# Vincentqyw/image-matching-webui

Hardware: AMD Instinct MI355X
Metric: image-pairs/sec @640x480 SuperPoint+LightGlue (higher is better)
Workload: dtype f32 via 3xf16 split MFMA, f32 accumulate; P.V of LightGlue's cross blocks in two products (audited per block: layer error <= 7.1e-6, score error <= 4.7e-5, profiles/r05_lab_attention_mix.txt)

## Files before the change

### image-matching-webui_amd/csrc/gemm_tile.h

```cpp
#pragma once
#include "gemm.h"

#define BM 128
#define BN 128

struct TileCtx {
    int M, N, row0, col0, seq, z;
    const float* bias;
    long wsel;
};

__device__ __forceinline__ bool gemm_tile_setup(const GemmP& p, TileCtx& c, int bn = BN, int bm = BM) {
    c.z = blockIdx.z;
    c.M = p.mcnt ? p.mcnt[c.z * p.cnt_stride] : p.M;
    c.N = p.ncnt ? p.ncnt[c.z * p.cnt_stride] : p.N;
    const int ncol = (p.N + bn - 1) / bn;
    const int tile = xcd_remap(blockIdx.x, gridDim.x);
    if (p.group_rows > 1) {
        const int nrow = (p.M + BM - 1) / BM;
        const int per = p.group_rows * ncol;
        const int g = tile / per, t = tile - g * per;
        const int rows = min(p.group_rows, nrow - g * p.group_rows);
        c.row0 = (g * p.group_rows + t % rows) * BM;
        c.col0 = (t / rows) * bn;
    } else {
        c.row0 = (tile / ncol) * bm;
        c.col0 = (tile % ncol) * bn;
    }
    if (c.row0 >= c.M || c.col0 >= c.N) return false;
    c.bias = p.bias;
    c.seq = 0;
    c.wsel = 0;
    if (p.rows_per_seq > 0) {
        c.seq = c.row0 / p.rows_per_seq;
        const int i0 = c.row0 - c.seq * p.rows_per_seq;
        if (p.cnt && i0 >= p.cnt[c.seq]) return false;
        if (p.active && p.active[c.seq >> 1] == 0) return false;
        if (p.wsel) {
            c.wsel = p.wsel[c.seq >> 1] + p.wsel_off;
            if (c.bias) c.bias += (size_t)c.wsel * p.b_stride;
        }
    }
    return true;
}
```

### image-matching-webui_amd/csrc/gemm_wreg.hip

```cpp
#include <stdlib.h>

#include "gemm.h"
#include "gemm_tile.h"

#define WR_BN 256
#ifdef WR_LAB
__device__ int wr_lab_flags = 0;
#define WR_FLAGS (__builtin_amdgcn_readfirstlane(wr_lab_flags))
#else
#define WR_FLAGS 0
#endif
#define WR_F_NOSTORE 1
#define WR_F_ONETILE 2
#define WR_F_NOEPI 4
#define WR_F_NOWLOAD 8
#define WR_F_NOXLOAD 16
#define WR_F_NOSTORE_V 32
#define WR_F_NOSTORE_QK 64
#define WR_F_STAGGER(f) (((f) >> 8) & 255)
#define WR_STG_ROW 68
#define WR_STG_TROW 36
#define WR_WAVE_LDS 9216

typedef unsigned int u32x4_t __attribute__((ext_vector_type(4)));
__device__ __forceinline__ const void* wr_uniform_ptr(const void* p) {
    const size_t v = (size_t)p;
    const unsigned lo32 = (unsigned)__builtin_amdgcn_readfirstlane((int)(unsigned)(v & 0xffffffffu));
    const unsigned hi32 = (unsigned)__builtin_amdgcn_readfirstlane((int)(unsigned)(v >> 32));
    return (const void*)((size_t)lo32 | ((size_t)hi32 << 32));
}
__device__ __forceinline__ void wr_wave_fence() {
    __builtin_amdgcn_s_waitcnt(0xc07f);
    __builtin_amdgcn_wave_barrier();
}

template <int EPI, bool SINGLE, bool PIPE = true, int MT = 4>
__global__ __launch_bounds__(256, 2) void gemm_wreg_kernel(GemmP p) {
    __shared__ uint4 smem[(4 * WR_WAVE_LDS) / 16];
    char* sm = reinterpret_cast<char*>(smem);
    const int tid = threadIdx.x;
    const int lane = tid & 63, wid = tid >> 6;
    const int lo = lane & 31, hi = lane >> 5;
    TileCtx c;
    if (!gemm_tile_setup(p, c, WR_BN, 32 * MT)) return;
    const float* A = p.A + (size_t)c.z * p.a_bs;
    const float wsc = p.wscale ? p.wscale[c.wsel] : 1.0f;
    const int labf = WR_FLAGS;
    if (WR_F_STAGGER(labf) != 0 && (int)blockIdx.x >= p.st_nct && (int)blockIdx.x < 4 * p.st_nct)
        for (int i = 0; i < WR_F_STAGGER(labf) * ((int)blockIdx.x / p.st_nct); ++i) __builtin_amdgcn_s_sleep(16);
    const int nkt = (labf & WR_F_ONETILE) ? 1 : p.K >> 5, nks = 2 * nkt;

    f32x16 acc[2][MT];
#pragma unroll
    for (int n = 0; n < 2; ++n)
#pragma unroll
        for (int m = 0; m < MT; ++m)
#pragma unroll
            for (int r = 0; r < 16; ++r) acc[n][m][r] = 0.0f;

    const int g = tid & 3;
    const int rl0 = tid >> 2, rl1 = 64 + (tid >> 2);
    const bool st0 = MT >= 2 || rl0 < 32, st1 = MT == 4;
    const int wo0 = (((g >> 1) * 4 + (rl0 >> 5)) * 64 + (g & 1) * 32 + ((rl0 & 31) ^ (2 * g))) * 16;
    const int wo1 = (((g >> 1) * 4 + (rl1 >> 5)) * 64 + (g & 1) * 32 + ((rl1 & 31) ^ (2 * g))) * 16;
    const float* pa0 = A + (size_t)min(c.row0 + (st0 ? rl0 : 0), c.M - 1) * p.lda + g * 8;
    const float* pa1 = A + (size_t)min(c.row0 + (st1 ? rl1 : 0), c.M - 1) * p.lda + g * 8;
    bool lnc = false;
    float mu0 = 0.f, mu1 = 0.f;
    if constexpr (EPI == EPI_QKV_VIT || EPI == EPI_CONV) {
        lnc = p.ln_stats != nullptr;
        if (lnc) {
            mu0 = p.ln_stats[2 * (size_t)min(c.row0 + (st0 ? rl0 : 0), c.M - 1)];
            mu1 = p.ln_stats[2 * (size_t)min(c.row0 + (st1 ? rl1 : 0), c.M - 1)];
        }
    }
    f32x4 xa0, xb0, xa1, xb1;
    auto issue = [&](int kt) __attribute__((always_inline)) {
        if (st0) {
            xa0 = *reinterpret_cast<const f32x4*>(pa0 + kt * 32);
            xb0 = *reinterpret_cast<const f32x4*>(pa0 + kt * 32 + 4);
        }
        if (st1) {
            xa1 = *reinterpret_cast<const f32x4*>(pa1 + kt * 32);
            xb1 = *reinterpret_cast<const f32x4*>(pa1 + kt * 32 + 4);
        }
    };
    auto store = [&](int stg) __attribute__((always_inline)) {
        uint4 h, l;
        if constexpr (EPI == EPI_QKV_VIT || EPI == EPI_CONV) {
            if (lnc) {
                xa0 -= mu0;
                xb0 -= mu0;
                xa1 -= mu1;
                xb1 -= mu1;
            }
        }
        if constexpr (SINGLE) {
            if (st0) *reinterpret_cast<uint4*>(sm + stg * 16384 + wo0) = half8_rtn(__builtin_bit_cast(float4, xa0), __builtin_bit_cast(float4, xb0));
            if (st1) *reinterpret_cast<uint4*>(sm + stg * 16384 + wo1) = half8_rtn(__builtin_bit_cast(float4, xa1), __builtin_bit_cast(float4, xb1));
            return;
        }
        if (st0) {
            split8(__builtin_bit_cast(float4, xa0), __builtin_bit_cast(float4, xb0), h, l);
            *reinterpret_cast<uint4*>(sm + stg * 16384 + wo0) = h;
            if constexpr (!SINGLE) *reinterpret_cast<uint4*>(sm + stg * 16384 + 8192 + wo0) = l;
        }
        if (st1) {
            split8(__builtin_bit_cast(float4, xa1), __builtin_bit_cast(float4, xb1), h, l);
            *reinterpret_cast<uint4*>(sm + stg * 16384 + wo1) = h;
            if constexpr (!SINGLE) *reinterpret_cast<uint4*>(sm + stg * 16384 + 8192 + wo1) = l;
        }
    };
    const int nfr = (p.N + 31) >> 5;
    const size_t plane_bytes = (size_t)nfr * 32 * p.K * 2;
    const __amdgpu_buffer_rsrc_t rWh =
        __builtin_amdgcn_make_buffer_rsrc(const_cast<void*>(wr_uniform_ptr(p.Wh + (size_t)c.wsel * p.w_stride)), 0, (unsigned)plane_bytes, 0x00020000);
    const __amdgpu_buffer_rsrc_t rWl =
        __builtin_amdgcn_make_buffer_rsrc(const_cast<void*>(wr_uniform_ptr(p.Wl + (size_t)c.wsel * p.w_stride)), 0, (unsigned)plane_bytes, 0x00020000);
    unsigned wof[2];
#pragma unroll
    for (int n = 0; n < 2; ++n) {
        const int nf = min((c.col0 >> 5) + 2 * wid + n, nfr - 1);
        wof[n] = (unsigned)((nf * (p.K >> 4)) * 64 + lane) * 16u;
    }
    uint4 wc[2][2], wn[2][2];
    auto loadw = [&](int s, uint4(&w)[2][2]) __attribute__((always_inline)) {
#pragma unroll
        for (int n = 0; n < 2; ++n) {
            const u32x4_t vh = __builtin_amdgcn_raw_buffer_load_b128(rWh, wof[n], (unsigned)s * 1024u, 0);
            w[n][0] = make_uint4(vh.x, vh.y, vh.z, vh.w);
            if constexpr (!SINGLE) {
                const u32x4_t vl = __builtin_amdgcn_raw_buffer_load_b128(rWl, wof[n], (unsigned)s * 1024u, 0);
                w[n][1] = make_uint4(vl.x, vl.y, vl.z, vl.w);
            }
        }
    };
    auto kstep = [&](int stg, int ks, uint4(&w)[2][2]) __attribute__((always_inline)) {
        const int apos = (hi * 32 + (lo ^ (2 * (2 * ks + hi)))) * 16;
#pragma unroll
        for (int mh = 0; mh < (MT + 1) / 2; ++mh) {
            constexpr int MH = MT >= 2 ? 2 : 1;
            uint4 ah[MH], al[MH];
#pragma unroll
            for (int m = 0; m < MH; ++m) {
                const int fo = stg * 16384 + (ks * 4 + 2 * mh + m) * 1024 + apos;
                ah[m] = *reinterpret_cast<const uint4*>(sm + fo);
                if constexpr (!SINGLE) al[m] = *reinterpret_cast<const uint4*>(sm + fo + 8192);
            }
#pragma unroll
            for (int n = 0; n < 2; ++n)
#pragma unroll
                for (int m = 0; m < MH; ++m) {
                    if constexpr (!SINGLE) {
                        acc[n][2 * mh + m] = mfma16(w[n][0], al[m], acc[n][2 * mh + m]);
                        acc[n][2 * mh + m] = mfma16(w[n][1], ah[m], acc[n][2 * mh + m]);
                    }
                    acc[n][2 * mh + m] = mfma16(w[n][0], ah[m], acc[n][2 * mh + m]);
                }
            if constexpr (PIPE) {
                if (mh == 0) __builtin_amdgcn_sched_barrier(0);
            }
        }
    };

    if constexpr (PIPE) {
        uint4 w0[2][2], w1[2][2], w2[2][2];
        issue(0);
        loadw(0, w0);
        if (nks > 1) loadw(1, w1);
        store(0);
        if (nkt > 1) issue(1);
        __syncthreads();
#define WR_TILE(KT, WA, WB, WC)                                  \
    {                                                            \
        const int kt_ = (KT), stg_ = kt_ & 1, s_ = 2 * kt_;      \
        if (s_ + 2 < nks && !(labf & WR_F_NOWLOAD)) loadw(s_ + 2, WC); \
        __builtin_amdgcn_sched_barrier(0);                       \
        kstep(stg_, 0, WA);                                      \
        __builtin_amdgcn_sched_barrier(0);                       \
        if (kt_ + 1 < nkt && !(labf & WR_F_NOXLOAD)) {           \
            store(stg_ ^ 1);                                     \
            if (kt_ + 2 < nkt) issue(kt_ + 2);                   \
        }                                                        \
        if (s_ + 3 < nks && !(labf & WR_F_NOWLOAD)) loadw(s_ + 3, WA); \
        __builtin_amdgcn_sched_barrier(0);                       \
        kstep(stg_, 1, WB);                                      \
        __syncthreads();                                         \
    }
        int kt = 0;
#pragma unroll 1
        for (; kt + 3 <= nkt; kt += 3) {
            WR_TILE(kt, w0, w1, w2)
            WR_TILE(kt + 1, w2, w0, w1)
            WR_TILE(kt + 2, w1, w2, w0)
        }
        if (kt < nkt) WR_TILE(kt, w0, w1, w2)
        if (kt + 1 < nkt) WR_TILE(kt + 1, w2, w0, w1)
#undef WR_TILE
    } else {
    issue(0);
    loadw(0, wc);
    store(0);
    if (nkt > 1) issue(1);
    __syncthreads();
#pragma unroll 1
    for (int kt = 0; kt < nkt; ++kt) {
        const int stg = kt & 1;
        loadw(2 * kt + 1, wn);
        kstep(stg, 0, wc);
        if (kt + 1 < nkt) {
            store(stg ^ 1);
            if (kt + 2 < nkt) issue(kt + 2);
            loadw(2 * kt + 2, wc);
        }
        kstep(stg, 1, wn);
        __syncthreads();
    }
    }

    float* st = reinterpret_cast<float*>(sm + wid * WR_WAVE_LDS);
    const int fw0 = c.col0 + 64 * wid;
    if (fw0 >= c.N) return;
    if (labf & WR_F_NOEPI) {
        if (acc[0][0][0] == 12345.678f) p.C[0] = acc[1][MT - 1][3];
        return;
    }
    bool do_store = !(labf & WR_F_NOSTORE);
    auto park_rows = [&](int m) __attribute__((always_inline)) {
#pragma unroll
        for (int n = 0; n < 2; ++n)
#pragma unroll
            for (int q = 0; q < 4; ++q)
                *reinterpret_cast<float4*>(st + lo * WR_STG_ROW + 32 * n + 8 * q + 4 * hi) =
                    make_float4(acc[n][m][4 * q + 0] * wsc, acc[n][m][4 * q + 1] * wsc, acc[n][m][4 * q + 2] * wsc, acc[n][m][4 * q + 3] * wsc);
    };
    if constexpr (EPI == EPI_QKV || EPI == EPI_CROSS || EPI == EPI_QKV_VIT) {
        const int CW = p.heads * 64;
        const int t = fw0 / CW, hd = (fw0 - t * CW) >> 6;
        float* dst;
        bool vt, rope, scale;
        if (EPI == EPI_QKV || EPI == EPI_QKV_VIT) {
            const int role = t + (EPI == EPI_QKV_VIT ? p.role0 : 0);
            dst = (role == 0) ? p.Q : (role == 1) ? p.Kt : p.V;
            vt = (role == 2);
            rope = (role < 2);
            scale = (role == 0);
        } else {
            dst = (t == 0) ? p.Q : p.V;
            vt = (t == 1);
            rope = false;
            scale = (t == 0);
        }
        unsigned short* d16 = reinterpret_cast<unsigned short*>(dst);
        if ((labf & WR_F_NOSTORE_V) && vt) do_store = false;
        if ((labf & WR_F_NOSTORE_QK) && !vt) do_store = false;
        const int R = p.rows_per_seq;
        const int i0 = c.row0 - c.seq * R;
        if (EPI == EPI_QKV_VIT && !vt) {
            const int tab0 = i0 + (p.rope_seq_row0 ? p.rope_seq_row0[c.seq] : 0);
            const int d0 = (lane & 7) * 8, dp = d0 ^ 16;
            const bool first = (d0 & 16) == 0;
            const int ti = (d0 >> 5) * 16 + (d0 & 8);
            float4 ba = make_float4(0.f, 0.f, 0.f, 0.f), bb = ba, pa = ba, pb = ba;
            if (c.bias != nullptr) {
                ba = *reinterpret_cast<const float4*>(c.bias + fw0 + d0);
                bb = *reinterpret_cast<const float4*>(c.bias + fw0 + d0 + 4);
                pa = *reinterpret_cast<const float4*>(c.bias + fw0 + dp);
                pb = *reinterpret_cast<const float4*>(c.bias + fw0 + dp + 4);
            }
#pragma unroll
            for (int m = 0; m < MT; ++m) {
                float4 tc[4][2], ts[4][2];
#pragma unroll
                for (int pass = 0; pass < 4; ++pass) {
                    const size_t ir = (size_t)(tab0 + 32 * m + pass * 8 + (lane >> 3)) * 32 + ti;
                    tc[pass][0] = *reinterpret_cast<const float4*>(p.rope_cos + ir);
                    tc[pass][1] = *reinterpret_cast<const float4*>(p.rope_cos + ir + 4);
                    ts[pass][0] = *reinterpret_cast<const float4*>(p.rope_sin + ir);
                    ts[pass][1] = *reinterpret_cast<const float4*>(p.rope_sin + ir + 4);
                }
                park_rows(m);
                wr_wave_fence();
#pragma unroll
                for (int pass = 0; pass < 4; ++pass) {
                    const int tl = pass * 8 + (lane >> 3);
                    const float4 va = *reinterpret_cast<const float4*>(st + tl * WR_STG_ROW + d0);
                    const float4 vb = *reinterpret_cast<const float4*>(st + tl * WR_STG_ROW + d0 + 4);
                    const float4 wa = *reinterpret_cast<const float4*>(st + tl * WR_STG_ROW + dp);
                    const float4 wb = *reinterpret_cast<const float4*>(st + tl * WR_STG_ROW + dp + 4);
                    float mine[8] = {va.x + ba.x, va.y + ba.y, va.z + ba.z, va.w + ba.w, vb.x + bb.x, vb.y + bb.y, vb.z + bb.z, vb.w + bb.w};
                    float part[8] = {wa.x + pa.x, wa.y + pa.y, wa.z + pa.z, wa.w + pa.w, wb.x + pb.x, wb.y + pb.y, wb.z + pb.z, wb.w + pb.w};
                    if (lnc) {
                        const float2 mr = *reinterpret_cast<const float2*>(p.ln_stats + 2 * (size_t)(c.row0 + 32 * m + tl));
                        const float xa[8] = {va.x, va.y, va.z, va.w, vb.x, vb.y, vb.z, vb.w}, xp[8] = {wa.x, wa.y, wa.z, wa.w, wb.x, wb.y, wb.z, wb.w};
                        const float ba8[8] = {ba.x, ba.y, ba.z, ba.w, bb.x, bb.y, bb.z, bb.w}, pa8[8] = {pa.x, pa.y, pa.z, pa.w, pb.x, pb.y, pb.z, pb.w};
#pragma unroll
                        for (int j = 0; j < 8; ++j) {
                            mine[j] = mr.y * xa[j] + ba8[j];
                            part[j] = mr.y * xp[j] + pa8[j];
                        }
                    }
                    const float cw[8] = {tc[pass][0].x, tc[pass][0].y, tc[pass][0].z, tc[pass][0].w, tc[pass][1].x, tc[pass][1].y, tc[pass][1].z, tc[pass][1].w};
                    const float ss[8] = {ts[pass][0].x, ts[pass][0].y, ts[pass][0].z, ts[pass][0].w, ts[pass][1].x, ts[pass][1].y, ts[pass][1].z, ts[pass][1].w};
                    float v[8];
#pragma unroll
                    for (int j = 0; j < 8; ++j) {
                        float x = mine[j], y = part[j];
                        asm volatile("" : "+v"(x), "+v"(y));
                        const float r = first ? __builtin_fmaf(x, cw[j], -(y * ss[j])) : __builtin_fmaf(x, cw[j], y * ss[j]);
                        v[j] = scale ? r * p.alpha : r;
                    }
                    uint4 hv, lv;
                    split8(make_float4(v[0], v[1], v[2], v[3]), make_float4(v[4], v[5], v[6], v[7]), hv, lv);
                    unsigned short* o = d16 + (((size_t)c.seq * p.heads + hd) * R + i0 + 32 * m + tl) * 64 + d0;
                    if (do_store) {
                        *reinterpret_cast<uint4*>(o) = hv;
                        *reinterpret_cast<uint4*>(o + p.plane_halves) = lv;
                    }
                }
                wr_wave_fence();
            }
        } else if (!vt) {
            const int d0 = (lane & 7) * 8;
            float4 ba = make_float4(0.f, 0.f, 0.f, 0.f), bb = ba;
            if (c.bias != nullptr) {
                ba = *reinterpret_cast<const float4*>(c.bias + fw0 + d0);
                bb = *reinterpret_cast<const float4*>(c.bias + fw0 + d0 + 4);
            }
            float4 tc[2][4], ts[2][4];
            auto load_tables = [&](int m, float4(&cs)[4], float4(&sn)[4]) __attribute__((always_inline)) {
#pragma unroll
                for (int pass = 0; pass < 4; ++pass) {
                    const size_t row = (size_t)(c.row0 + 32 * m + pass * 8 + (lane >> 3));
                    cs[pass] = *reinterpret_cast<const float4*>(p.rope_cos + row * 32 + (d0 >> 1));
                    sn[pass] = *reinterpret_cast<const float4*>(p.rope_sin + row * 32 + (d0 >> 1));
                }
            };
            if (rope) load_tables(0, tc[0], ts[0]);
#pragma unroll
            for (int m = 0; m < MT; ++m) {
                park_rows(m);
                wr_wave_fence();
                if (rope && m + 1 < MT) load_tables(m + 1, tc[(m + 1) & 1], ts[(m + 1) & 1]);
#pragma unroll
                for (int pass = 0; pass < 4; ++pass) {
                    const int tl = pass * 8 + (lane >> 3);
                    const float4 va = *reinterpret_cast<const float4*>(st + tl * WR_STG_ROW + d0);
                    const float4 vb = *reinterpret_cast<const float4*>(st + tl * WR_STG_ROW + d0 + 4);
                    float v[8] = {va.x + ba.x, va.y + ba.y, va.z + ba.z, va.w + ba.w, vb.x + bb.x, vb.y + bb.y, vb.z + bb.z, vb.w + bb.w};
                    if (rope) {
                        const float4 cs = tc[m & 1][pass], sn = ts[m & 1][pass];
                        const float cw[4] = {cs.x, cs.y, cs.z, cs.w}, ss[4] = {sn.x, sn.y, sn.z, sn.w};
#pragma unroll
                        for (int j = 0; j < 4; ++j) {
                            float a0 = v[2 * j], a1 = v[2 * j + 1];
                            asm volatile("" : "+v"(a0), "+v"(a1));
                            v[2 * j] = __builtin_fmaf(a0, cw[j], -(a1 * ss[j]));
                            v[2 * j + 1] = __builtin_fmaf(a1, cw[j], a0 * ss[j]);
                        }
                    }
                    if (scale) {
#pragma unroll
                        for (int j = 0; j < 8; ++j) v[j] *= p.alpha;
                    }
                    uint4 hv, lv;
                    split8(make_float4(v[0], v[1], v[2], v[3]), make_float4(v[4], v[5], v[6], v[7]), hv, lv);
                    unsigned short* o = d16 + (((size_t)c.seq * p.heads + hd) * R + i0 + 32 * m + tl) * 64 + d0;
                    if (do_store) {
                        *reinterpret_cast<uint4*>(o) = hv;
                        *reinterpret_cast<uint4*>(o + p.plane_halves) = lv;
                    }
                }
                wr_wave_fence();
            }
        } else {
#pragma unroll
            for (int m = 0; m < MT; ++m) {
#pragma unroll
                for (int n = 0; n < 2; ++n)
#pragma unroll
                    for (int r = 0; r < 16; ++r) st[(32 * n + 8 * (r >> 2) + 4 * hi + (r & 3)) * WR_STG_TROW + lo] = acc[n][m][r] * wsc;
                wr_wave_fence();
#pragma unroll
                for (int pass = 0; pass < 4; ++pass) {
                    const int d = pass * 16 + (lane >> 2), tk = (lane & 3) * 8;
                    const float bd = c.bias ? c.bias[fw0 + d] : 0.0f;
                    float4 va = *reinterpret_cast<const float4*>(st + d * WR_STG_TROW + tk);
                    float4 vb = *reinterpret_cast<const float4*>(st + d * WR_STG_TROW + tk + 4);
                    if (lnc) {
                        const float4* ms4 = reinterpret_cast<const float4*>(p.ln_stats + 2 * (size_t)(c.row0 + 32 * m + tk));
                        const float4 q0 = ms4[0], q1 = ms4[1], q2 = ms4[2], q3 = ms4[3];
                        va = make_float4(q0.y * va.x, q0.w * va.y, q1.y * va.z, q1.w * va.w);
                        vb = make_float4(q2.y * vb.x, q2.w * vb.y, q3.y * vb.z, q3.w * vb.w);
                    }
                    uint4 hv, lv;
                    split8(make_float4(va.x + bd, va.y + bd, va.z + bd, va.w + bd), make_float4(vb.x + bd, vb.y + bd, vb.z + bd, vb.w + bd), hv, lv);
                    unsigned short* o = d16 + (((size_t)c.seq * p.heads + hd) * 64 + d) * R + i0 + 32 * m + tk;
                    if (do_store) {
                        *reinterpret_cast<uint4*>(o) = hv;
                        *reinterpret_cast<uint4*>(o + p.plane_halves) = lv;
                    }
                }
                wr_wave_fence();
            }
        }
    } else {
        float* C = p.C + (size_t)c.z * p.c_bs;
        const int fl = (lane & 15) * 4;
        const int f0 = fw0 + fl;
        float4 b4 = make_float4(0.f, 0.f, 0.f, 0.f);
        if (c.bias != nullptr) b4 = *reinterpret_cast<const float4*>(c.bias + f0);
#pragma unroll
        for (int m = 0; m < MT; ++m) {
            park_rows(m);
            wr_wave_fence();
#pragma unroll
            for (int pass = 0; pass < 8; ++pass) {
                const int tl = pass * 4 + (lane >> 4);
                const int row = c.row0 + 32 * m + tl;
                if (row < c.M) {
                    float4 t4 = *reinterpret_cast<const float4*>(st + tl * WR_STG_ROW + fl);
                    if (lnc) {
                        const float rs = p.ln_stats[2 * (size_t)row + 1];
                        t4 = make_float4(rs * t4.x, rs * t4.y, rs * t4.z, rs * t4.w);
                    }
                    float v[4] = {t4.x + b4.x, t4.y + b4.y, t4.z + b4.z, t4.w + b4.w};
                    float* dstp = C + (size_t)row * p.ldc + f0;
                    if (EPI == EPI_CONV) {
                        if (p.resid != nullptr) {
                            const float4 r4 = *reinterpret_cast<const float4*>(p.resid + (size_t)row * p.ldr + f0);
                            v[0] += r4.x;
                            v[1] += r4.y;
                            v[2] += r4.z;
                            v[3] += r4.w;
                        }
                        if (p.act == 1) {
#pragma unroll
                            for (int j = 0; j < 4; ++j) v[j] = fmaxf(v[j], 0.0f);
                        } else if (p.act == 2) {
#pragma unroll
                            for (int j = 0; j < 4; ++j) v[j] = v[j] > 0.0f ? v[j] : 0.01f * v[j];
                        } else if (p.act == 3) {
#pragma unroll
                            for (int j = 0; j < 4; ++j) v[j] = gelu_poly(v[j]);
                        }
                    } else if (EPI == EPI_BIAS) {
#pragma unroll
                        for (int j = 0; j < 4; ++j) v[j] *= p.alpha;
                    } else if (EPI == EPI_RELU) {
#pragma unroll
                        for (int j = 0; j < 4; ++j) v[j] = fmaxf(v[j], 0.0f);
                    } else if (EPI == EPI_RESID) {
                        const float4 o4 = *reinterpret_cast<const float4*>(dstp);
                        v[0] += o4.x;
                        v[1] += o4.y;
                        v[2] += o4.z;
                        v[3] += o4.w;
                    }
                    if (do_store) *reinterpret_cast<float4*>(dstp) = make_float4(v[0], v[1], v[2], v[3]);
                }
            }
            wr_wave_fence();
        }
    }
}

bool gemm_wreg_ok(const imcui_hip_s* h, const GemmP& p) {
    const int mode = h ? h->opt[OPT_GEMM_WREG] : 2;
    if (mode == 0 || (mode == 1 && p.epi != EPI_QKV && p.epi != EPI_CROSS && p.epi != EPI_QKV_VIT) || p.Wh == nullptr || p.Wl == nullptr || p.A2 != nullptr || p.conv_k > 0 || p.batch != 1 || p.mcnt || p.ncnt || p.group_rows > 1 ||
        p.rup_h > 0)
        return false;
    if (p.K % 32 != 0 || p.N % 64 != 0 || (p.lda & 3) != 0) return false;
    if (p.ln_stats != nullptr && p.epi != EPI_QKV_VIT && p.epi != EPI_CONV) return false;
    if (p.epi == EPI_QKV_VIT)
        return p.split_out && p.v_transposed && p.heads % 4 == 0 && p.N % (p.heads * 64) == 0 && p.rows_per_seq > 0 && p.rows_per_seq % 128 == 0 && p.M % 128 == 0 && !p.single;
    if (p.epi == EPI_QKV || p.epi == EPI_CROSS)
        return p.split_out && p.v_transposed && p.heads == 4 && p.N % 256 == 0 && p.rows_per_seq > 0 && p.rows_per_seq % 128 == 0 && p.M % 128 == 0;
    if (p.single && p.epi != EPI_CONV) return false;
    if ((p.ldc & 3) != 0 || (p.epi == EPI_CONV && p.resid != nullptr && (p.ldr & 3) != 0)) return false;
    return p.epi == EPI_BIAS || p.epi == EPI_RELU || p.epi == EPI_RESID || p.epi == EPI_CONV;
}

template <int EPI, int MT>
static void wreg_launch_small(imcui_hip_s* h, const GemmP& p, hipStream_t stream) {
    gemm_route_note(h, MT == 2 ? GR_WREG_MT2 : GR_WREG_MT1, EPI);
    hipLaunchKernelGGL((gemm_wreg_kernel<EPI, false, true, MT>), dim3(cdiv(p.M, 32 * MT) * cdiv(p.N, WR_BN), 1, 1), dim3(256), 0, stream, p);
}
static int wreg_tile_tokens(const imcui_hip_s* h, const GemmP& p) {
    if (p.epi != EPI_QKV && p.epi != EPI_CROSS && p.epi != EPI_BIAS && p.epi != EPI_CONV) return 128;
    if (p.single || p.group_rows > 1 || (h && h->opt[OPT_WREG_PIPE] == 0)) return 128;
    const int forced = h ? h->opt[OPT_WREG_TILE] : 0;
    if (forced == 128 || forced == 64 || forced == 32) return forced;
    const long ncol = cdiv(p.N, WR_BN);
    if ((long)cdiv(p.M, 128) * ncol >= 256) return 128;
    if ((long)cdiv(p.M, 64) * ncol >= 256) return 64;
    return 32;
}
template <bool PIPE>
static void wreg_launch(imcui_hip_s* h, const GemmP& p, hipStream_t stream) {
    const dim3 grid(cdiv(p.M, BM) * cdiv(p.N, WR_BN), 1, 1);
    const int kind = PIPE ? GR_WREG_PIPE : GR_WREG_ROLLED;
    switch (p.epi) {
        case EPI_BIAS: gemm_route_note(h, kind, EPI_BIAS); hipLaunchKernelGGL((gemm_wreg_kernel<EPI_BIAS, false, PIPE>), grid, dim3(256), 0, stream, p); break;
        case EPI_RELU: gemm_route_note(h, kind, EPI_RELU); hipLaunchKernelGGL((gemm_wreg_kernel<EPI_RELU, false, PIPE>), grid, dim3(256), 0, stream, p); break;
        case EPI_RESID: gemm_route_note(h, kind, EPI_RESID); hipLaunchKernelGGL((gemm_wreg_kernel<EPI_RESID, false, PIPE>), grid, dim3(256), 0, stream, p); break;
        case EPI_QKV: gemm_route_note(h, kind, EPI_QKV); hipLaunchKernelGGL((gemm_wreg_kernel<EPI_QKV, false, PIPE>), grid, dim3(256), 0, stream, p); break;
        case EPI_CROSS: gemm_route_note(h, kind, EPI_CROSS); hipLaunchKernelGGL((gemm_wreg_kernel<EPI_CROSS, false, PIPE>), grid, dim3(256), 0, stream, p); break;
        case EPI_QKV_VIT: gemm_route_note(h, kind, EPI_QKV_VIT); hipLaunchKernelGGL((gemm_wreg_kernel<EPI_QKV_VIT, false, PIPE>), grid, dim3(256), 0, stream, p); break;
        default:
            if (p.single) {
                gemm_route_note(h, PIPE ? GR_WREG_PIPE_SINGLE : GR_WREG_ROLLED_SINGLE, EPI_CONV);
                hipLaunchKernelGGL((gemm_wreg_kernel<EPI_CONV, true, PIPE>), grid, dim3(256), 0, stream, p);
            } else {
                gemm_route_note(h, kind, EPI_CONV);
                hipLaunchKernelGGL((gemm_wreg_kernel<EPI_CONV, false, PIPE>), grid, dim3(256), 0, stream, p);
            }
    }
}
void gemm_wreg_launch(imcui_hip_s* h, const GemmP& p, hipStream_t stream) {
    const int tok = wreg_tile_tokens(h, p);
    if (tok != 128) {
        if (p.epi == EPI_QKV)
            tok == 64 ? wreg_launch_small<EPI_QKV, 2>(h, p, stream) : wreg_launch_small<EPI_QKV, 1>(h, p, stream);
        else if (p.epi == EPI_CROSS)
            tok == 64 ? wreg_launch_small<EPI_CROSS, 2>(h, p, stream) : wreg_launch_small<EPI_CROSS, 1>(h, p, stream);
        else if (p.epi == EPI_CONV)
            tok == 64 ? wreg_launch_small<EPI_CONV, 2>(h, p, stream) : wreg_launch_small<EPI_CONV, 1>(h, p, stream);
        else
            tok == 64 ? wreg_launch_small<EPI_BIAS, 2>(h, p, stream) : wreg_launch_small<EPI_BIAS, 1>(h, p, stream);
        return;
    }
    if (h && h->opt[OPT_WREG_PIPE] == 0)
        wreg_launch<false>(h, p, stream);
    else
        wreg_launch<true>(h, p, stream);
}
```

Before: 976.9.

## Pair two 128-row tiles per 512-thread block sharing an LDS weight ring

For pipelined QKV and cross-attention projections, each 512-thread block now covers two adjacent 128-row tiles. Both halves share weight fragments that are DMA'd straight into a three-slot LDS ring with global_load_lds, so each weight tile is read from global memory once per pair instead of once per tile and the per-wave register weight loads go away. This adds a large shared-memory footprint at one block per CU, inline asm with manual m0 and vmcnt handling, and a per-step block-wide barrier. It also halves the grid, which can reduce occupancy for small token counts.

```diff
diff --git a/image-matching-webui_amd/csrc/gemm_tile.h b/image-matching-webui_amd/csrc/gemm_tile.h
--- a/image-matching-webui_amd/csrc/gemm_tile.h
+++ b/image-matching-webui_amd/csrc/gemm_tile.h
@@ -10,7 +10,7 @@
     long wsel;
 };
 
-__device__ __forceinline__ bool gemm_tile_setup(const GemmP& p, TileCtx& c, int bn = BN, int bm = BM) {
+__device__ __forceinline__ bool gemm_tile_setup(const GemmP& p, TileCtx& c, int bn = BN, int bm = BM, int roff = 0) {
     c.z = blockIdx.z;
     c.M = p.mcnt ? p.mcnt[c.z * p.cnt_stride] : p.M;
     c.N = p.ncnt ? p.ncnt[c.z * p.cnt_stride] : p.N;
@@ -24,7 +24,7 @@
         c.row0 = (g * p.group_rows + t % rows) * BM;
         c.col0 = (t / rows) * bn;
     } else {
-        c.row0 = (tile / ncol) * bm;
+        c.row0 = (tile / ncol) * bm + roff;
         c.col0 = (tile % ncol) * bn;
     }
     if (c.row0 >= c.M || c.col0 >= c.N) return false;
diff --git a/image-matching-webui_amd/csrc/gemm_wreg.hip b/image-matching-webui_amd/csrc/gemm_wreg.hip
--- a/image-matching-webui_amd/csrc/gemm_wreg.hip
+++ b/image-matching-webui_amd/csrc/gemm_wreg.hip
@@ -21,6 +21,8 @@
 #define WR_STG_ROW 68
 #define WR_STG_TROW 36
 #define WR_WAVE_LDS 9216
+#define WR_RING_SLOT 32768
+#define WR_PAIR_LDS (65536 + 3 * WR_RING_SLOT)
 
 typedef unsigned int u32x4_t __attribute__((ext_vector_type(4)));
 __device__ __forceinline__ const void* wr_uniform_ptr(const void* p) {
@@ -34,17 +36,35 @@
     __builtin_amdgcn_wave_barrier();
 }
 
-template <int EPI, bool SINGLE, bool PIPE = true, int MT = 4>
-__global__ __launch_bounds__(256, 2) void gemm_wreg_kernel(GemmP p) {
-    __shared__ uint4 smem[(4 * WR_WAVE_LDS) / 16];
+template <int EPI, bool SINGLE, bool PIPE = true, int MT = 4, bool PAIR = false>
+__global__ __launch_bounds__(PAIR ? 512 : 256, PAIR ? 1 : 2) void gemm_wreg_kernel(GemmP p) {
+    static_assert(!PAIR || (PIPE && MT == 4 && !SINGLE), "the pair tile is the pipelined 128-token split-arithmetic loop");
+    __shared__ uint4 smem[(PAIR ? WR_PAIR_LDS : 4 * WR_WAVE_LDS) / 16];
     char* sm = reinterpret_cast<char*>(smem);
     const int tid = threadIdx.x;
     const int lane = tid & 63, wid = tid >> 6;
     const int lo = lane & 31, hi = lane >> 5;
+    const int half = PAIR ? wid >> 2 : 0;
+    const int wf = wid & 3;
+    const int ht = tid & 255;
+    char* sa = sm + half * 32768;
     TileCtx c;
-    if (!gemm_tile_setup(p, c, WR_BN, 32 * MT)) return;
+    bool live = true;
+    long wsel = 0;
+    if constexpr (PAIR) {
+        TileCtx c0, c1;
+        const bool l0 = gemm_tile_setup(p, c0, WR_BN, 256, 0);
+        const bool l1 = gemm_tile_setup(p, c1, WR_BN, 256, 128);
+        if (!l0 && !l1) return;
+        c = half ? c1 : c0;
+        live = half ? l1 : l0;
+        wsel = l0 ? c0.wsel : c1.wsel;
+    } else {
+        if (!gemm_tile_setup(p, c, WR_BN, 32 * MT)) return;
+        wsel = c.wsel;
+    }
     const float* A = p.A + (size_t)c.z * p.a_bs;
-    const float wsc = p.wscale ? p.wscale[c.wsel] : 1.0f;
+    const float wsc = p.wscale ? p.wscale[wsel] : 1.0f;
     const int labf = WR_FLAGS;
     if (WR_F_STAGGER(labf) != 0 && (int)blockIdx.x >= p.st_nct && (int)blockIdx.x < 4 * p.st_nct)
         for (int i = 0; i < WR_F_STAGGER(labf) * ((int)blockIdx.x / p.st_nct); ++i) __builtin_amdgcn_s_sleep(16);
@@ -58,8 +78,8 @@
 #pragma unroll
             for (int r = 0; r < 16; ++r) acc[n][m][r] = 0.0f;
 
-    const int g = tid & 3;
-    const int rl0 = tid >> 2, rl1 = 64 + (tid >> 2);
+    const int g = ht & 3;
+    const int rl0 = ht >> 2, rl1 = 64 + (ht >> 2);
     const bool st0 = MT >= 2 || rl0 < 32, st1 = MT == 4;
     const int wo0 = (((g >> 1) * 4 + (rl0 >> 5)) * 64 + (g & 1) * 32 + ((rl0 & 31) ^ (2 * g))) * 16;
     const int wo1 = (((g >> 1) * 4 + (rl1 >> 5)) * 64 + (g & 1) * 32 + ((rl1 & 31) ^ (2 * g))) * 16;
@@ -96,27 +116,27 @@
             }
         }
         if constexpr (SINGLE) {
-            if (st0) *reinterpret_cast<uint4*>(sm + stg * 16384 + wo0) = half8_rtn(__builtin_bit_cast(float4, xa0), __builtin_bit_cast(float4, xb0));
-            if (st1) *reinterpret_cast<uint4*>(sm + stg * 16384 + wo1) = half8_rtn(__builtin_bit_cast(float4, xa1), __builtin_bit_cast(float4, xb1));
+            if (st0) *reinterpret_cast<uint4*>(sa + stg * 16384 + wo0) = half8_rtn(__builtin_bit_cast(float4, xa0), __builtin_bit_cast(float4, xb0));
+            if (st1) *reinterpret_cast<uint4*>(sa + stg * 16384 + wo1) = half8_rtn(__builtin_bit_cast(float4, xa1), __builtin_bit_cast(float4, xb1));
             return;
         }
         if (st0) {
             split8(__builtin_bit_cast(float4, xa0), __builtin_bit_cast(float4, xb0), h, l);
-            *reinterpret_cast<uint4*>(sm + stg * 16384 + wo0) = h;
-            if constexpr (!SINGLE) *reinterpret_cast<uint4*>(sm + stg * 16384 + 8192 + wo0) = l;
+            *reinterpret_cast<uint4*>(sa + stg * 16384 + wo0) = h;
+            if constexpr (!SINGLE) *reinterpret_cast<uint4*>(sa + stg * 16384 + 8192 + wo0) = l;
         }
         if (st1) {
             split8(__builtin_bit_cast(float4, xa1), __builtin_bit_cast(float4, xb1), h, l);
-            *reinterpret_cast<uint4*>(sm + stg * 16384 + wo1) = h;
-            if constexpr (!SINGLE) *reinterpret_cast<uint4*>(sm + stg * 16384 + 8192 + wo1) = l;
+            *reinterpret_cast<uint4*>(sa + stg * 16384 + wo1) = h;
+            if constexpr (!SINGLE) *reinterpret_cast<uint4*>(sa + stg * 16384 + 8192 + wo1) = l;
         }
     };
     const int nfr = (p.N + 31) >> 5;
     const size_t plane_bytes = (size_t)nfr * 32 * p.K * 2;
     const __amdgpu_buffer_rsrc_t rWh =
-        __builtin_amdgcn_make_buffer_rsrc(const_cast<void*>(wr_uniform_ptr(p.Wh + (size_t)c.wsel * p.w_stride)), 0, (unsigned)plane_bytes, 0x00020000);
+        __builtin_amdgcn_make_buffer_rsrc(const_cast<void*>(wr_uniform_ptr(p.Wh + (size_t)wsel * p.w_stride)), 0, (unsigned)plane_bytes, 0x00020000);
     const __amdgpu_buffer_rsrc_t rWl =
-        __builtin_amdgcn_make_buffer_rsrc(const_cast<void*>(wr_uniform_ptr(p.Wl + (size_t)c.wsel * p.w_stride)), 0, (unsigned)plane_bytes, 0x00020000);
+        __builtin_amdgcn_make_buffer_rsrc(const_cast<void*>(wr_uniform_ptr(p.Wl + (size_t)wsel * p.w_stride)), 0, (unsigned)plane_bytes, 0x00020000);
     unsigned wof[2];
 #pragma unroll
     for (int n = 0; n < 2; ++n) {
@@ -135,6 +155,39 @@
             }
         }
     };
+    typedef __attribute__((address_space(3))) void* lptr_t;
+    const int wid_s = __builtin_amdgcn_readfirstlane(wid);
+    const unsigned ring_lds = __builtin_amdgcn_readfirstlane((unsigned)(size_t)(lptr_t)(sm + 65536)) + (unsigned)wid_s * 4096u;
+    const char* gwh = reinterpret_cast<const char*>(p.Wh + (size_t)wsel * p.w_stride) + ((size_t)((c.col0 >> 5) + wid_s) * nks * 64 + lane) * 16;
+    const char* gwl = reinterpret_cast<const char*>(p.Wl + (size_t)wsel * p.w_stride) + ((size_t)((c.col0 >> 5) + wid_s) * nks * 64 + lane) * 16;
+    auto dma_ring = [&](int kt, int slot) __attribute__((always_inline)) {
+        const char* h0 = gwh + (size_t)kt * 2048;
+        const char* l0 = gwl + (size_t)kt * 2048;
+        const unsigned dst = ring_lds + (unsigned)slot * (unsigned)WR_RING_SLOT;
+        unsigned keep;
+        asm volatile("s_mov_b32 %0, m0\n\t"
+                     "s_mov_b32 m0, %5\n\ts_nop 0\n\tglobal_load_lds_dwordx4 %1, off\n\t"
+                     "s_mov_b32 m0, %6\n\ts_nop 0\n\tglobal_load_lds_dwordx4 %2, off\n\t"
+                     "s_mov_b32 m0, %7\n\ts_nop 0\n\tglobal_load_lds_dwordx4 %3, off\n\t"
+                     "s_mov_b32 m0, %8\n\ts_nop 0\n\tglobal_load_lds_dwordx4 %4, off\n\t"
+                     "s_mov_b32 m0, %0"
+                     : "=&s"(keep)
+                     : "v"(h0), "v"(l0), "v"(h0 + 1024), "v"(l0 + 1024), "s"(dst), "s"(dst + 1024u), "s"(dst + 2048u), "s"(dst + 3072u)
+                     : "memory");
+    };
+    auto wait_ring = [&](bool younger) __attribute__((always_inline)) {
+        if (younger)
+            asm volatile("s_waitcnt vmcnt(8)" ::: "memory");
+        else
+            asm volatile("s_waitcnt vmcnt(0)" ::: "memory");
+    };
+    auto ring_w = [&](int slot, int ks, uint4(&w)[2][2]) __attribute__((always_inline)) {
+#pragma unroll
+        for (int n = 0; n < 2; ++n)
+#pragma unroll
+            for (int pl = 0; pl < 2; ++pl)
+                w[n][pl] = *reinterpret_cast<const uint4*>(sm + 65536 + slot * WR_RING_SLOT + (((2 * wf + n) * 2 + ks) * 2 + pl) * 1024 + lane * 16);
+    };
     auto kstep = [&](int stg, int ks, uint4(&w)[2][2]) __attribute__((always_inline)) {
         const int apos = (hi * 32 + (lo ^ (2 * (2 * ks + hi)))) * 16;
 #pragma unroll
@@ -144,8 +197,8 @@
 #pragma unroll
             for (int m = 0; m < MH; ++m) {
                 const int fo = stg * 16384 + (ks * 4 + 2 * mh + m) * 1024 + apos;
-                ah[m] = *reinterpret_cast<const uint4*>(sm + fo);
-                if constexpr (!SINGLE) al[m] = *reinterpret_cast<const uint4*>(sm + fo + 8192);
+                ah[m] = *reinterpret_cast<const uint4*>(sa + fo);
+                if constexpr (!SINGLE) al[m] = *reinterpret_cast<const uint4*>(sa + fo + 8192);
             }
 #pragma unroll
             for (int n = 0; n < 2; ++n)
@@ -163,7 +216,49 @@
         }
     };
 
-    if constexpr (PIPE) {
+    if constexpr (PAIR) {
+        dma_ring(0, 0);
+        if (nkt > 1) dma_ring(1, 1);
+        issue(0);
+        store(0);
+        if (nkt > 1) {
+            issue(1);
+            asm volatile("s_waitcnt vmcnt(4)" ::: "memory");
+        } else {
+            wait_ring(false);
+        }
+        __syncthreads();
+#define WR_PAIR_TILE(KT, SLOT)                                        \
+    {                                                                 \
+        const int kt_ = (KT), stg_ = kt_ & 1;                         \
+        uint4 w_[2][2];                                               \
+        ring_w(SLOT, 0, w_);                                          \
+        kstep(stg_, 0, w_);                                           \
+        __builtin_amdgcn_sched_barrier(0);                            \
+        if (kt_ + 1 < nkt) {                                          \
+            store(stg_ ^ 1);                                          \
+            if (kt_ + 2 < nkt) {                                      \
+                dma_ring(kt_ + 2, ((SLOT) + 2) % 3);                   \
+                issue(kt_ + 2);                                       \
+            }                                                         \
+        }                                                             \
+        __builtin_amdgcn_sched_barrier(0);                            \
+        ring_w(SLOT, 1, w_);                                          \
+        kstep(stg_, 1, w_);                                           \
+        wait_ring(kt_ + 2 < nkt);                                     \
+        __syncthreads();                                              \
+    }
+        int kt = 0;
+#pragma unroll 1
+        for (; kt + 3 <= nkt; kt += 3) {
+            WR_PAIR_TILE(kt, 0)
+            WR_PAIR_TILE(kt + 1, 1)
+            WR_PAIR_TILE(kt + 2, 2)
+        }
+        if (kt < nkt) WR_PAIR_TILE(kt, 0)
+        if (kt + 1 < nkt) WR_PAIR_TILE(kt + 1, 1)
+#undef WR_PAIR_TILE
+    } else if constexpr (PIPE) {
         uint4 w0[2][2], w1[2][2], w2[2][2];
         issue(0);
         loadw(0, w0);
@@ -219,7 +314,8 @@
     }
 
     float* st = reinterpret_cast<float*>(sm + wid * WR_WAVE_LDS);
-    const int fw0 = c.col0 + 64 * wid;
+    const int fw0 = c.col0 + 64 * wf;
+    if (!live) return;
     if (fw0 >= c.N) return;
     if (labf & WR_F_NOEPI) {
         if (acc[0][0][0] == 12345.678f) p.C[0] = acc[1][MT - 1][3];
@@ -499,13 +595,26 @@
 template <bool PIPE>
 static void wreg_launch(imcui_hip_s* h, const GemmP& p, hipStream_t stream) {
     const dim3 grid(cdiv(p.M, BM) * cdiv(p.N, WR_BN), 1, 1);
+    const dim3 pair_grid(cdiv(p.M, 2 * BM) * cdiv(p.N, WR_BN), 1, 1);
     const int kind = PIPE ? GR_WREG_PIPE : GR_WREG_ROLLED;
     switch (p.epi) {
         case EPI_BIAS: gemm_route_note(h, kind, EPI_BIAS); hipLaunchKernelGGL((gemm_wreg_kernel<EPI_BIAS, false, PIPE>), grid, dim3(256), 0, stream, p); break;
         case EPI_RELU: gemm_route_note(h, kind, EPI_RELU); hipLaunchKernelGGL((gemm_wreg_kernel<EPI_RELU, false, PIPE>), grid, dim3(256), 0, stream, p); break;
         case EPI_RESID: gemm_route_note(h, kind, EPI_RESID); hipLaunchKernelGGL((gemm_wreg_kernel<EPI_RESID, false, PIPE>), grid, dim3(256), 0, stream, p); break;
-        case EPI_QKV: gemm_route_note(h, kind, EPI_QKV); hipLaunchKernelGGL((gemm_wreg_kernel<EPI_QKV, false, PIPE>), grid, dim3(256), 0, stream, p); break;
-        case EPI_CROSS: gemm_route_note(h, kind, EPI_CROSS); hipLaunchKernelGGL((gemm_wreg_kernel<EPI_CROSS, false, PIPE>), grid, dim3(256), 0, stream, p); break;
+        case EPI_QKV:
+            gemm_route_note(h, kind, EPI_QKV);
+            if (PIPE)
+                hipLaunchKernelGGL((gemm_wreg_kernel<EPI_QKV, false, true, 4, true>), pair_grid, dim3(512), 0, stream, p);
+            else
+                hipLaunchKernelGGL((gemm_wreg_kernel<EPI_QKV, false, false>), grid, dim3(256), 0, stream, p);
+            break;
+        case EPI_CROSS:
+            gemm_route_note(h, kind, EPI_CROSS);
+            if (PIPE)
+                hipLaunchKernelGGL((gemm_wreg_kernel<EPI_CROSS, false, true, 4, true>), pair_grid, dim3(512), 0, stream, p);
+            else
+                hipLaunchKernelGGL((gemm_wreg_kernel<EPI_CROSS, false, false>), grid, dim3(256), 0, stream, p);
+            break;
         case EPI_QKV_VIT: gemm_route_note(h, kind, EPI_QKV_VIT); hipLaunchKernelGGL((gemm_wreg_kernel<EPI_QKV_VIT, false, PIPE>), grid, dim3(256), 0, stream, p); break;
         default:
             if (p.single) {
```

Result: no change. 979.0 (median of 6 runs) (+0.2%).
